# indianajohn/akaze-rust

Hardware: AMD Instinct MI355X
Metric: Mpix/s through extract_features (4 oct x 4 sub) (higher is better)
Workload: dtype f32

## Files before the change

### akaze-rust_amd/csrc/akz_api.cpp

```cpp
#include "akz_ctx.hpp"

unsigned akz::host_cpu_share() {
    unsigned n = std::max(1u, std::thread::hardware_concurrency());
    cpu_set_t set;
    if (sched_getaffinity(0, sizeof(set), &set) == 0) n = std::max(1, CPU_COUNT(&set));
    if (FILE* f = fopen("/sys/fs/cgroup/cpu.max", "r")) {
        char q[32] = {0};
        long period = 0;
        if (fscanf(f, "%31s %ld", q, &period) == 2 && period > 0 && strcmp(q, "max") != 0)
            n = std::min<unsigned>(n, (unsigned)std::max(1L, atol(q) / period));
        fclose(f);
    }
    if (const char* e = std::getenv("LOCAL_WORLD_SIZE")) {
        const int ranks = atoi(e);
        if (ranks > 1) n = std::max(2u, n / (unsigned)ranks);
    }
    return std::max(1u, n);
}

int level_info_out(const std::vector<LevelPlan>& plan, uint64_t level, double* etime, double* esigma,
                          uint32_t* octave, uint32_t* sublevel, uint32_t* sigma_size, uint32_t* lw, uint32_t* lh,
                          uint32_t* det_sigma, uint64_t* n_tau, double* tau, uint64_t tau_cap) {
    if (level >= plan.size()) {
        set_error("level out of range");
// ... 64 lines not shown
int akz_stream_create(int device, void** stream_out) {
    if (!stream_out) return AKZ_ERR_INVALID_ARG;
    AKZ_HIP_TRY(hipSetDevice(device));
    hipStream_t s = nullptr;
    AKZ_HIP_TRY(hipStreamCreateWithFlags(&s, hipStreamNonBlocking));
    *stream_out = (void*)s;
    return AKZ_OK;
}
int akz_stream_destroy(int device, void* stream) {
    AKZ_HIP_TRY(hipSetDevice(device));
    if (stream) AKZ_HIP_TRY(hipStreamDestroy((hipStream_t)stream));
    return AKZ_OK;
}

int akz_ctx_destroy(akz_ctx* c) {
    if (!c) return AKZ_OK;
    (void)hipSetDevice(c->device);
    finisher_stop(c);
    for (akz_ctx* l : c->lanes) (void)akz_ctx_destroy(l);
    c->lanes.clear();
    if (c->lane_in) { (void)hipEventDestroy(c->lane_in); c->lane_in = nullptr; }
    (void)hipStreamSynchronize(c->stream);
    DevBuf* bufs[] = {&c->lazy[0], &c->lazy[1], &c->lazy[2], &c->lazy[3], &c->lazy[4], &c->lazy[5],
                      &c->scratch[0], &c->scratch[1], &c->scratch[2], &c->scratch[3], &c->scratch[4], &c->scratch[5], &c->scratch_coarse,
                      &c->small, &c->cand, &c->cand_sorted, &c->sort_scratch, &c->rel_scratch, &c->sel_scratch, &c->sel_recs, &c->bucket_scratch, &c->kp_in, &c->kp_out, &c->match_a, &c->match_b, &c->match_rec, &c->match_state,
                      &c->match_out, &c->cosi, &c->mm_q8, &c->mm_t8, &c->mm_pop, &c->mm_tab, &c->mm_cols,
                      &c->ms1.q8, &c->ms1.t8, &c->ms1.pop, &c->ms1.tab, &c->ms1.cols, &c->ms1.rec, &c->ransac_dev,
                      &c->mp_in, &c->mp_raw, &c->mp_tab, &c->mp_trials, &c->mp_keep, &c->gd_tab, &c->gd_rec, &c->gd_out, &c->cx_rev, &c->kn_part, &c->kn_io};
    for (DevBuf* b : bufs)
        if (b->p) (void)hipFree(b->p);
    for (DevBuf* b : {&c->jpeg_coef, &c->jpeg_plane, &c->jpeg_frames})
        if (b->p) (void)hipFree(b->p);
    for (int k = 0; k < akz_ctx::kJpegSlots; ++k) {
        if (c->jpeg_up[k]) (void)hipEventDestroy(c->jpeg_up[k]);
        if (c->jpeg_pin[k].p) (void)hipHostFree(c->jpeg_pin[k].p);
    }
    for (DevBuf& b : c->fetch_tmp)
        if (b.p) (void)hipFree(b.p);
    for (auto& set : c->fetch_out)
        for (DevBuf& b : set)
            if (b.p) (void)hipFree(b.p);
    if (c->fetch_stage.p) (void)hipHostFree(c->fetch_stage.p);
    for (hipEvent_t* e : {&c->fetch_chunk[0], &c->fetch_chunk[1], &c->fetch_chunk[2], &c->fetch_chunk[3], &c->fetch_start,
                          &c->fetch_join, &c->fetch_ready[0], &c->fetch_ready[1], &c->fetch_free[0], &c->fetch_free[1]}) {
        if (*e) (void)hipEventDestroy(*e);
        *e = nullptr;
    }
// ... 274 lines not shown
int akz_ctx_set_candidate_hint(akz_ctx* c, uint32_t per_image) {
    AKZ_TRY(bind(c));
    c->cand_cap_hint = std::max<uint32_t>(per_image, 16u);
    for (akz_ctx* l : c->lanes) l->cand_cap_hint = c->cand_cap_hint.load();
    return AKZ_OK;
}
int akz_ctx_set_match_mode(akz_ctx* c, int mode) {
    AKZ_TRY(bind(c));
    if (mode < 0 || mode > 3) return AKZ_ERR_INVALID_ARG;
    c->match_mode = mode;
    for (akz_ctx* l : c->lanes) l->match_mode = mode;
    return AKZ_OK;
}
int akz_ctx_set_fed_mode(akz_ctx* c, int mode) {
    AKZ_TRY(bind(c));
    if (mode != 0 && mode != 2) return AKZ_ERR_INVALID_ARG;
    c->fed_mode = mode;
    for (akz_ctx* l : c->lanes) l->fed_mode = mode;
    return AKZ_OK;
}
const char* akz_fed_kernel_name(void) { return "k_level_march + k_fed_own"; }
int akz_debug_march_bands(int kind, uint32_t w, uint32_t h, uint32_t n, int half_width, int32_t* rows, uint32_t cap,
                          uint32_t* n_bands) {
    if (!n_bands || (cap && !rows) || kind < 0 || kind > 1 || w < 16 || h < 16 || n == 0 || half_width < 1 || half_width > 4)
        return AKZ_ERR_INVALID_ARG;
    *n_bands = launch::march_band_rows(kind, w, h, n, half_width, rows, cap);
    return AKZ_OK;
}
int akz_debug_detector_set_cells(int half_width, const uint32_t* w, const uint32_t* h, uint32_t n_entries, uint32_t n, int32_t* cells,
                                 uint32_t cap, int32_t* grids, uint32_t* n_workgroups) {
    if (!n_workgroups || !w || !h || !grids || (cap && !cells) || n_entries < 1 || n_entries > launch::detector_march_set_max() || n == 0 ||
        half_width < 1 || half_width > 4)
        return AKZ_ERR_INVALID_ARG;
    for (uint32_t e = 0; e < n_entries; ++e)
        if (w[e] < 4u * (uint32_t)half_width + 8u || h[e] < 4u * (uint32_t)half_width + 8u) return AKZ_ERR_INVALID_ARG;
    *n_workgroups = launch::detector_set_cells(half_width, w, h, n_entries, n, cells, cap, grids);
    return AKZ_OK;
}
const char* akz_detector_kernel_name(void) { return "detector (k_detector_march + k_detector_tiled)"; }
int akz_debug_set_schedule(akz_ctx* c, int key, int value) {
    if (!c || key < 0 || key > 11) return AKZ_ERR_INVALID_ARG;
    AKZ_TRY(bind(c));
    c->sched[key] = value;
    if (key == 7 || key == 8) launch::march_min_band_rows(c->sched[7], c->sched[8]);
    if (key == 11) launch::detector_set_waves(value >= 11 && value <= 14 ? value - 10 : 0);
    if (key == 4) {
        c->big_px_sync = value > 0 ? (uint64_t)value * 1000u : gates::kBigPxSync;
        c->big_px_async = value > 0 ? (uint64_t)value * 1000u : gates::kBigPxAsync;
        c->lane_px = value > 0 ? (uint64_t)value * 1000u : gates::kLanePx;
        for (akz_ctx* l : c->lanes) {
            l->big_px_sync = std::max(c->big_px_sync, c->lane_px);
            l->big_px_async = std::max(c->big_px_async, c->lane_px);
        }
    }
    return AKZ_OK;
}
int akz_debug_placement_verdict(float spin_pair_ms, float tiny_pair_ms, float tiny_alone_ms, float spin_ms) {
    return akz::placement_verdict(spin_pair_ms, tiny_pair_ms, tiny_alone_ms, spin_ms);
}
int akz_debug_stream_placement(akz_ctx* c, int* info) {
    if (!c || !info) return AKZ_ERR_INVALID_ARG;
    AKZ_TRY(bind(c));
    info[0] = c->placed ? 1 : 0;
    info[1] = c->pre_mode;
// ... 90 lines not shown
```

### akaze-rust_amd/csrc/akz_ctx.hpp

```cpp
#pragma once
#include <algorithm>
#include <cmath>
#include <cstdlib>
#include <cstddef>
#include <cstring>
#include <atomic>
#include <condition_variable>
#include <functional>
#include <map>
#include <memory>
#include <mutex>
#include <thread>
#include <sched.h>
#include <time.h>
#include <type_traits>

#include "akz_internal.hpp"
#include "akz_select.hpp"
#include "akz_pool.hpp"
#include "akz_gates.hpp"

#define AKZ_LOCAL __attribute__((visibility("hidden")))

namespace akz {
// ... 25 lines not shown
    bool quit = false;
};

enum Pin {
    PIN_LIST = 0,
    PIN_COUNT_SUMS,
    PIN_ROWS,
    PIN_PARAMS,
    PIN_COSI,
    PIN_CONTRAST,
    PIN_REL,
    PIN_REL_FLAGS,
    PIN_SEL_HDR,
    PIN_SPARE,
    PIN_COUNT_
};
struct akz_ctx {
    int device = 0;
    hipStream_t stream = nullptr;
    hipStream_t main = nullptr;
    bool own_stream = false;
    DevBuf scratch[6];
    DevBuf scratch_coarse;
    DevBuf lazy[6];
    DevBuf small;
    void* small_zero_p = nullptr;
    size_t small_zero = 0;
    DevBuf cand;
    DevBuf cand_sorted, sort_scratch;
    DevBuf rel_scratch;
    DevBuf sel_scratch, sel_recs;
    DevBuf bucket_scratch;
    int dbg_select = -1;
    std::atomic<uint32_t> last_total_kp{0};
    std::atomic<int> sel_last_mode{-1};
    std::atomic<int> sel_skip{0};
    std::atomic<uint64_t> sel_skip_shape{0};
    std::atomic<uint32_t> sel_last_ticks[4];
    std::atomic<uint32_t> sel_last_rounds{0}, sel_last_fallback{0};
    DevBuf kp_in, kp_out;
    DevBuf match_a, match_b, match_rec, match_out;
    DevBuf match_state;
    uint32_t match_epoch = 0;
    DevBuf ransac_dev, ransac_pin;
    DevBuf mp_in, mp_raw, mp_tab, mp_trials, mp_keep;
    DevBuf mp_pin_in, mp_pin_tab, mp_pin_smp[2], mp_pin_out;
// ... 34 lines not shown
    std::atomic<uint32_t> cand_cap_hint{1u << 15};
    std::atomic<int> live_results{0};
    bool dead = false;
    std::atomic<uint32_t> last_total_cands{0};
    std::atomic<uint64_t> last_cand_shape{0};
    hipStream_t aux = nullptr;
    std::mutex aux_m;
    hipStream_t coarse = nullptr;
    hipStream_t pre = nullptr;
    hipEvent_t pre_done = nullptr;
    hipStream_t copy = nullptr;
    DevBuf stage[kSlots];
    hipEvent_t staged[kSlots] = {nullptr, nullptr, nullptr};
    std::vector<akz_ctx*> lanes;
    unsigned next_lane = 0;
    bool is_lane = false;
    bool eager_finish = true;
    std::shared_ptr<Finisher> fin;
    hipEvent_t lane_in = nullptr;
    uint64_t stream_min_px = gates::kStreamPx;
    int prep_mode = 2;
    int det_mode = 2;
    int fed_mode = 2;
    int sched[12] = {0, 1, 0, 0, 0, 0, 0, 0, 0, 0, 0, 0};
    uint64_t big_px = gates::kBigPxAsync;
    uint64_t big_px_sync = gates::kBigPxSync, big_px_async = gates::kBigPxAsync;
    uint64_t lane_px = gates::kLanePx;
    static constexpr uint64_t kLaunchMarchPx = gates::kMarchPx;
    uint64_t launch_min_px = kLaunchMarchPx;
    bool placed = false;
    int pre_mode = 0;
    int place_replaced = 0;
    int place_collisions = 0;
    int place_retries = 0;
    int lane_collisions = 0;
    hipEvent_t probe_ev[2] = {nullptr, nullptr};
    int profiling = 0;
    akz_profile prof{};
    struct Span { int stage; hipEvent_t a, b; int row; };
    std::vector<Span> spans;
    std::vector<akz_kernel_row> rows;
    std::vector<hipEvent_t> ev_pool;
    std::mutex ev_m;
    static constexpr int kFedRing = 4;
    hipEvent_t fed_ev[kFedRing] = {nullptr, nullptr, nullptr, nullptr};
    hipEvent_t pre_ev[kFedRing] = {nullptr, nullptr, nullptr, nullptr};
    std::atomic<uint64_t> begin_seq{0};
// ... 276 lines not shown
```

### akaze-rust_amd/csrc/akz_extract_begin.cpp

```cpp
#include "akz_extract.hpp"

namespace {
enum class Prep : uint8_t {
    Tiled,
    Stream,
    LevelMarch,
    Resident
};
enum class Det : uint8_t {
    Fallback,
    NmsFused,
    TiledSet,
    March
};
struct BeginRoute {
    bool big = false;
    int prep_mode = 0;
    int pre_on = 0;
    bool level1_clone = false;
    size_t res_first = 0;
    size_t fork_level = 0;
    size_t oct1 = 0;
    bool own_kernels = true;
    struct Level {
        Prep prep = Prep::Tiled;
        uint32_t n1 = 0, rem = 0;
        bool fold_half = false;
        bool may_ride = false;
        Det det = Det::Fallback;
    };
    std::vector<Level> lv;
};

BeginRoute begin_route(const akz_ctx* c, const std::vector<LevelPlan>& plan, const akz_config& cfg, uint32_t w, uint32_t h, uint32_t n,
                       uint32_t flags, bool input_ready, bool big) {
    const size_t L = plan.size();
    BeginRoute rt;
    rt.big = big;
    rt.prep_mode = c->prep_mode;
    rt.lv.resize(L);
    const int pre_mode = c->sched[0] == 0 ? c->pre_mode : c->sched[0] == 1 ? 2 : c->sched[0] == 2 ? 1 : 0;
    if ((input_ready || (flags & AKZ_INPUT_READY)) && pre_mode != 0 && c->profiling < 2 && c->prep_mode == 2 && big &&
        launch::blur5_march_supported(w, h, (uint32_t)gaussian_kernel_size((float)cfg.base_scale_offset)) &&
        launch::contrast_march_supported(w, h, (uint32_t)gaussian_kernel_size(1.0f), (uint32_t)cfg.contrast_factor_num_bins))
        rt.pre_on = pre_mode;
    rt.level1_clone = L > 1 && plan[1].octave == plan[0].octave && plan[1].w == w && plan[1].h == h;
    const int fork_octave = c->sched[3] > 0 ? c->sched[3] : 2;
    rt.res_first = L;
    if (c->fed_mode == 2 && (c->prep_mode == 3 || (c->prep_mode == 2 && big))) {
        size_t f = 1;
// ... 24 lines not shown
        const LevelPlan& lv = plan[l];
        BeginRoute::Level& q = rt.lv[l];
        const int fam = detector_family(c, lv.det_sigma, lv.w, lv.h, n, border_margin(lv, cfg), (flags & AKZ_KEEP_ALL_PLANES) != 0);
        q.det = fam == 5 ? Det::March : fam == 4 ? Det::TiledSet : launch::detector_nms_fused_supported(lv.det_sigma) ? Det::NmsFused : Det::Fallback;
        if (l >= rt.fork_level && q.det == Det::Fallback) rt.own_kernels = false;
        if (l == 0) continue;
        const LevelPlan& pv = plan[l - 1];
        const bool half = lv.octave > pv.octave;
        const uint64_t lpx = (uint64_t)lv.w * lv.h * n;
        if (l >= rt.res_first) {
            q.prep = Prep::Resident;
        } else if (!lv.tau.empty() && c->fed_mode == 2 && launch::level_march_supported(lv.w, lv.h) &&
                   (c->prep_mode == 3 || (c->prep_mode == 2 && lpx >= gates::kLevelMarchPx))) {
            q.prep = Prep::LevelMarch;
            q.n1 = std::min<uint32_t>((uint32_t)lv.tau.size(), 4u);
            q.rem = (uint32_t)lv.tau.size() - q.n1;
            q.fold_half = half && launch::level_march_half_supported(lv.w, lv.h, pv.w, pv.h, q.n1);
        } else if (c->prep_mode != 0 && launch::prep_stream_supported(lv.w, lv.h) &&
                   (c->prep_mode == 1 || (c->prep_mode >= 2 && !half && lpx >= c->stream_min_px))) {
            q.prep = Prep::Stream;
        }
        q.may_ride = c->sched[6] == 0 && c->fed_mode == 2 && lv.octave == pv.octave && q.prep == Prep::Tiled;
    }
    return rt;
}

struct BeginState {
    akz_ctx* c;
    akz_result* r;
    const BeginRoute& rt;
    uint32_t n;
    bool keep_all;
    hipStream_t s;
    hipStream_t ls;
    uint64_t seq;
    Candidate* d_cand;
    uint32_t* d_count;
    uint32_t cap;
    std::vector<float> g1;
    std::vector<char> det_done;
    std::vector<char> prepared;
    bool head_fused = false;
    float* P(size_t l, int p) const { return r->planes[l][p]; }
    size_t L() const { return r->plan.size(); }
};

// ... 70 lines not shown
                                           (uint32_t)plan[l].tau.size(), ht[l].data(), plan[l].octave});
        px_steps += (uint64_t)plan[l].w * plan[l].h * b.n * plan[l].tau.size();
    }
    StageTimer st(c, AKZ_ST_FED);
    st.kernel(AKZ_KR_OCTAVE_RESIDENT, (uint32_t)rl.size(), plan[i].w, plan[i].h, b.n, 1, 0, px_steps);
    launch::octave_resident(b.ls, b.P(i - 1, AKZ_LT), plan[i - 1].w, plan[i - 1].h, b.n, rl.data(), (uint32_t)rl.size(), b.g1.data(), b.r->d_k);
    if (c->profiling) {
        c->prof.fed_launches += 1;
        c->prof.fed_px_steps += px_steps;
    }
    AKZ_HIP_TRY(hipGetLastError());
    return AKZ_OK;
}

int level_by_march(BeginState& b, size_t i, float* A, float* B) {
    akz_ctx* c = b.c;
    const LevelPlan &lv = b.r->plan[i], &pv = b.r->plan[i - 1];
    const BeginRoute::Level& q = b.rt.lv[i];
    const uint32_t n = b.n, n1 = q.n1, rem = q.rem;
    const bool half = lv.octave > pv.octave;
    const uint32_t rest = rem ? fed_num_launches(c, rem, lv.w, lv.h, n) : 0;
    float* d1 = fed_dst(rest + 1, 1, A, B);
    const float* level_in = b.P(i - 1, AKZ_LT);
    if (half && !q.fold_half) {
        StageTimer st(c, AKZ_ST_PREP);
        float* hb = d1 == A ? B : A;
        launch::half_size(b.ls, b.P(i - 1, AKZ_LT), hb, pv.w, pv.h, n);
        level_in = hb;
    }
    float ht[4];
    for (uint32_t j = 0; j < n1; ++j) ht[j] = 0.5f * (float)lv.tau[j];
    {
        StageTimer st(c, AKZ_ST_FED);
        st.kernel(AKZ_KR_LEVEL_MARCH, n1 | (q.fold_half ? 16u : 0u) | ((rem == 0 && b.keep_all) ? 32u : 0u), lv.w, lv.h, n, 1,
                  (uint64_t)lv.w * lv.h * n, (uint64_t)lv.w * lv.h * n * n1);
        launch::level_march(b.ls, level_in, b.P(i, AKZ_LSMOOTH), b.P(i, AKZ_LFLOW), d1,
                            (rem == 0 && b.keep_all) ? b.P(i, AKZ_LSTEP) : nullptr, lv.w, lv.h, n, b.g1.data(), b.r->d_k,
                            lv.octave, ht, n1, q.fold_half ? pv.w : 0u, q.fold_half ? pv.h : 0u);
        if (c->profiling) {
            c->prof.fed_launches += 1;
            c->prof.fed_px_steps += (uint64_t)lv.w * lv.h * n * n1;
            c->prof.fused_px += (uint64_t)lv.w * lv.h * n;
        }
    }
    if (rem) {
        StageTimer st(c, AKZ_ST_FED);
        st.kernel(AKZ_KR_FED_OWN, rem, lv.w, lv.h, n, rest, 0, (uint64_t)lv.w * lv.h * n * rem);
        AKZ_TRY(fed_impl(c, d1, A, B, b.P(i, AKZ_LFLOW), b.keep_all ? b.P(i, AKZ_LSTEP) : nullptr, lv.w, lv.h, n, lv.tau.data() + n1, rem));
    }
    AKZ_HIP_TRY(hipGetLastError());
    return AKZ_OK;
}

int level_by_launches(BeginState& b, size_t i, float* A, float* B) {
    akz_ctx* c = b.c;
    const LevelPlan &lv = b.r->plan[i], &pv = b.r->plan[i - 1];
    const uint32_t n = b.n, n_tau = (uint32_t)lv.tau.size();
    const bool half = lv.octave > pv.octave;
    const float* fed_in = b.P(i - 1, AKZ_LT);
    float* half_buf = nullptr;
    if (half) {
// ... 184 lines not shown
    if (!c->fed_ev[0])
        for (hipEvent_t& e : c->fed_ev) AKZ_HIP_TRY(hipEventCreateWithFlags(&e, hipEventDisableTiming));
    if (!c->pre_ev[0])
        for (hipEvent_t& e : c->pre_ev) AKZ_HIP_TRY(hipEventCreateWithFlags(&e, hipEventDisableTiming));
    const uint64_t seq = c->begin_seq.load() + 1;
    struct StreamRestore {
        akz_ctx* c;
        hipStream_t main;
        ~StreamRestore() { c->stream = main; }
    } stream_restore{c, s};
    struct PrepModeRestore {
        akz_ctx* c;
        int mode;
        ~PrepModeRestore() { c->prep_mode = mode; }
    } prep_mode_restore{c, c->prep_mode};
    if (c->prep_mode == 2 && c->sched[6] == 0 && (uint64_t)w * h * n < gates::kTiledPrepPx) c->prep_mode = 0;
    const bool big = (uint64_t)w * h * n >= c->big_px;
    c->launch_min_px = big ? std::min<uint64_t>(akz_ctx::kLaunchMarchPx, (uint64_t)w * h * n) : akz_ctx::kLaunchMarchPx;
    if (big && !c->placed) AKZ_TRY(place_streams(c));
    const BeginRoute rt = begin_route(c, r->plan, r->cfg, w, h, n, flags, input_ready != nullptr, big);
    BeginState b{c, r, rt, n, keep_all, s, s, seq, (Candidate*)c->cand_slot[o.slot].p, (uint32_t*)c->count_slot[o.slot].p, cap,
                 {}, std::vector<char>(L, 0), std::vector<char>(L + 1, 0)};

    AKZ_TRY(level0<T>(b, d_imgs, input_ready));
    AKZ_TRY(ensure(c, c->scratch[5], plane_bytes(w, h, n)));
    b.g1 = gaussian_kernel(1.0f, gaussian_kernel_size(1.0f));
    AKZ_TRY(run_levels(b, 1, rt.oct1));
    AKZ_HIP_TRY(hipEventRecord(c->pre_ev[seq % akz_ctx::kFedRing], s));
    AKZ_TRY(run_levels(b, rt.oct1, rt.fork_level));
    AKZ_HIP_TRY(hipEventRecord(c->fed_ev[seq % akz_ctx::kFedRing], s));
    c->begin_seq.store(seq);

    hipStream_t done_on = s;
    if (rt.fork_level < L) AKZ_TRY(fork_and_join(b, &done_on));
    else AKZ_TRY(detectors(b, 0, L, s));
    AKZ_HIP_TRY(hipGetLastError());
    job->nms_done = StageTimer::get(c);
    AKZ_HIP_TRY(hipEventRecord(job->nms_done, done_on));
    job->done_stream = done_on;
    job->seq = seq;
    *out = o.keep(cap);
    return AKZ_OK;
}
template int extract_begin<uint8_t>(akz_ctx*, const uint8_t*, uint32_t, uint32_t, uint32_t, const akz_config*, uint32_t, akz_job**, int, hipEvent_t, bool);
template int extract_begin<float>(akz_ctx*, const float*, uint32_t, uint32_t, uint32_t, const akz_config*, uint32_t, akz_job**, int, hipEvent_t, bool);
```

### akaze-rust_amd/csrc/akz_internal.hpp

```cpp
#pragma once
#include <hip/hip_runtime.h>

#include <cstdint>
#include <functional>
#include <string>
#include <vector>

#include "../../include/akaze_hip.h"
#include "../../include/akaze_hip_debug.h"

namespace akz {

void set_error(const std::string& msg);
unsigned host_cpu_share();

using TrialsOnDevice = std::function<int(const float*, const float*, const float*, const float*, uint32_t, const uint32_t*, uint32_t,
                                         float, float, float*, int32_t*)>;
int remove_outliers_impl(const akz_keypoint* keypoints_0, uint64_t n0, const akz_keypoint* keypoints_1, uint64_t n1,
                         const akz_match* matches, uint64_t n_matches, uint64_t num_trials, float epsilon_model,
                         float epsilon_inlier, akz_match* out, uint64_t* n_out, const TrialsOnDevice& trials_on_device);

#define AKZ_HIP_TRY(expr)                                                                          \
    do {                                                                                           \
        hipError_t _e = (expr);                                                                    \
// ... 183 lines not shown
void detector_march(hipStream_t s, const float* lsmooth, uint32_t sigma, float* lx, float* ly, float* lxx, float* lyy,
                    float* lxy, float* ldet_out, uint32_t w, uint32_t h, uint32_t n, uint32_t level, float thr,
                    float border_m, Candidate* d_cand, uint32_t cap, uint32_t* d_count);
uint32_t detector_march_set_max();
void detector_march_set(hipStream_t s, uint32_t sigma, const DetLevelDesc* levels, uint32_t nlevels, uint32_t n, float thr,
                        Candidate* d_cand, uint32_t cap, uint32_t* d_count);
void detector_set_waves(int waves);
uint32_t detector_set_cells(int S, const uint32_t* w, const uint32_t* h, uint32_t nlv, uint32_t n, int32_t* cells, uint32_t cap,
                            int32_t* grids);
bool head_fused_supported(uint32_t w, uint32_t h, uint32_t ntaps0, uint32_t ntaps1);
void head_fused_u8(hipStream_t s, const uint8_t* in, float* lt0, float* blurred, float* gx, float* gy, uint32_t w, uint32_t h, uint32_t n,
                   const float* k5, const float* g3, unsigned long long* d_smax_bits, uint32_t* d_zero_word = nullptr);
void head_fused_f32(hipStream_t s, const float* in, float* lt0, float* blurred, float* gx, float* gy, uint32_t w, uint32_t h, uint32_t n,
                    const float* k5, const float* g3, unsigned long long* d_smax_bits, uint32_t* d_zero_word = nullptr);
void contrast_hist_final(hipStream_t s, const float* gx, const float* gy, uint32_t w, uint32_t h, uint32_t n, unsigned long long* d_smax_bits,
                         uint32_t nbins, uint32_t* d_hist, uint32_t* d_done, double percentile, double* d_k);
void flow_from_pair(hipStream_t s, const float* gx, const float* gy, float* lflow, uint32_t w, uint32_t h, uint32_t n, const double* d_k,
                    uint32_t k_pow);
void march_min_band_rows(int detector, int level);
bool level_march_supported(uint32_t w, uint32_t h);
bool level_march_half_supported(uint32_t w, uint32_t h, uint32_t pw, uint32_t ph, uint32_t n_steps);
void level_march(hipStream_t s, const float* prev, float* lsmooth, float* lflow, float* lt_out, float* lstep, uint32_t w,
                 uint32_t h, uint32_t n, const float* g3, const double* d_k, uint32_t k_pow, const float* half_taus,
                 uint32_t n_steps, uint32_t pw = 0, uint32_t ph = 0);
struct ResidentLevel {
    float *lt, *lsmooth, *lflow, *lstep;
    uint32_t w, h;
    bool half;
    uint32_t n_tau;
    const float* half_tau;
    uint32_t k_pow;
};
constexpr int kResidentMaxLevels = 10;
constexpr int kResidentMaxSteps = 448;
bool octave_resident_supported(uint32_t w, uint32_t h);
void octave_resident(hipStream_t s, const float* prev, uint32_t pw, uint32_t ph, uint32_t n, const ResidentLevel* levels,
                     uint32_t n_levels, const float* g3, const double* d_k);
bool detector_nms_fused_supported(uint32_t sigma);
void detector_nms_fused(hipStream_t s, const float* lsmooth, uint32_t sigma, float* lx, float* ly, float* lxx,
                        float* lyy, float* lxy, float* ldet_out, uint32_t w, uint32_t h, uint32_t n, uint32_t level,
                        float thr, float border_m, Candidate* d_cand, uint32_t cap, uint32_t* d_count);
void rcp_f64_to_f32(hipStream_t s, const double* x, float* out, uint64_t n);
void accumulate(hipStream_t s, float* a, const float* b, uint64_t count);
void ldet(hipStream_t s, const float* lxx, const float* lyy, const float* lxy, float* out, uint64_t count,
          float sigma_quat);
size_t sort_candidates_scratch(uint32_t cap, uint64_t max_px, uint32_t n_levels, uint32_t n_images);
uint32_t sort_small_capacity();
// ... 154 lines not shown
```

### akaze-rust_amd/csrc/akz_march.hip

```cpp
#include <hip/hip_runtime.h>

#include <algorithm>
#include <cstdlib>
#include <type_traits>

#include "akz_internal.hpp"
#include "akz_pm_g2.hpp"

namespace akz {
namespace {

typedef float f2 __attribute__((ext_vector_type(2)));
typedef float f2u __attribute__((ext_vector_type(2), aligned(4)));

constexpr int MT = 256;
constexpr int MW = 2 * MT;
constexpr int HALO = 16;
constexpr int USE = MW - 2 * HALO;
constexpr int PAD = 8;
constexpr int ROW = MW + 2 * PAD;
constexpr int CBUF = 32;
#ifndef AKZ_MARCH_PF
#define AKZ_MARCH_PF 3
#endif
// ... 373 lines not shown
        }
    }
    if (NMS) cands_flush(cbuf, cnum, nms, lane);
}

struct LevelTaus {
    float half_tau[4];
};
__device__ __forceinline__ f2 lds2(const float* p) { return f2{p[0], p[1]}; }
__device__ __forceinline__ f2 tap3(f2 a, f2 b, f2 c, float k0, float k1, float k2) {
    const f2 z = {0.0f, 0.0f};
    return ((z + k0 * a) + k1 * b) + k2 * c;
}
__device__ __forceinline__ double octave_contrast(double k, unsigned pow) {
    for (unsigned i = 0; i < pow; ++i) k = k * 0.75;
    return k;
}

typedef unsigned u4m __attribute__((ext_vector_type(4)));
template <int N, bool KEEPSTEP, bool ODDW, bool HALF = false>
__global__ void __launch_bounds__(MT, 3)
k_level_march(const float* __restrict__ prev, float* __restrict__ lsmooth_out, float* __restrict__ lflow_out,
              float* __restrict__ lt_out, float* __restrict__ lstep_out, int w, int h, MarchGrid g, float g0, float g1,
              float g2, float kn, float kwn, const double* __restrict__ d_k, unsigned k_pow, LevelTaus ht, int pw = 0, int ph = 0) {
    static_assert(!(HALF && ODDW), "the 2x2 mean is folded in for even level widths only");
    static_assert(N >= 1 && N <= 4, "fused diffusion steps");
    static_assert(N + 3 <= HALO, "strip halo");
    constexpr int NPL = 3 + N;
#ifndef AKZ_LEVEL_PF
#define AKZ_LEVEL_PF 2
#endif
    constexpr int PF = AKZ_LEVEL_PF;
    static_assert(PF >= 1 && PF <= 3, "prefetch ring");
    __shared__ __attribute__((aligned(16))) float s_row[2][NPL][ROW];
    const int tid = threadIdx.x;
    const int per = g.nbands * g.nstrips;
    const int cell = march_cell();
    if (cell >= g.total) return;
    const int img = __builtin_amdgcn_readfirstlane(cell / per);
    const int rem = cell - img * per;
    const int band = __builtin_amdgcn_readfirstlane(rem / g.nstrips), strip = rem - band * g.nstrips;
    int cs, ce;
    level_band_rows(g, band, h, &cs, &ce);
    if (cs >= ce) return;
    const int lt0 = cs == 1 ? 0 : cs, lt1 = ce == h - 1 ? h : ce;

    const int X0 = strip * USE - HALO;
    const int p0 = (2 * tid + HALO) & (MW - 1);
    const bool inner = p0 >= HALO && p0 < MW - HALO;
    const Cols C = make_cols(X0 + p0, inner, w);
    const int i0 = PAD + clampi(clampi(C.x0, 1, w - 2) - X0, 0, MW - 1) - 1;
    const int i1 = PAD + clampi(clampi(C.x0 + 1, 1, w - 2) - X0, 0, MW - 1) - 1;
    const int wi = PAD + p0;
    const bool edge_h = __ballot(i0 != wi - 1 || i1 != wi) != 0ull;
    const bool hxn0 = C.x0 > 0, hxp0 = C.x0 + 1 < w, hxn1 = C.x0 + 1 > 0, hxp1 = C.x0 + 2 < w;
    const bool edge_col = __ballot(!(hxn0 && hxp0 && hxn1 && hxp1)) != 0ull;

    const size_t base = (size_t)img * (size_t)w * (size_t)h;
    const __amdgpu_buffer_rsrc_t in = HALF ? plane_rsrc(prev + (size_t)img * (size_t)pw * (size_t)ph, pw, ph) : plane_rsrc(prev + base, w, h);
    const __amdgpu_buffer_rsrc_t o_ls[1] = {plane_rsrc(lsmooth_out + base, w, h)};
    const __amdgpu_buffer_rsrc_t o_lf[1] = {plane_rsrc(lflow_out + base, w, h)};
    __amdgpu_buffer_rsrc_t o_lt[KEEPSTEP ? 2 : 1];
    o_lt[0] = plane_rsrc(lt_out + base, w, h);
    if (KEEPSTEP) o_lt[1] = plane_rsrc(lstep_out + base, w, h);
    const __amdgpu_buffer_rsrc_t(&o_ltc)[KEEPSTEP ? 2 : 1] = o_lt;
    const double kc = octave_contrast(d_k[img], k_pow);
    const double inverse_k = 1.0 / (kc * kc);

    const int v0 = lt0 - N - 2;
    const int T = (lt1 - lt0) + 2 * N + 6;
    struct Fed {
        f2 v;
        u4m top, bot;
    };
    auto feed = [&](int t) -> Fed {
        Fed f;
        const unsigned row = (unsigned)clampi(v0 + min(t, T - 1), 0, h - 1);
        if constexpr (HALF) {
            const unsigned ro = 2u * row * ((unsigned)pw * 4u);
            f.top = __builtin_amdgcn_raw_buffer_load_b128(in, (int)(2u * C.vo_ld), (int)ro, 0);
            f.bot = __builtin_amdgcn_raw_buffer_load_b128(in, (int)(2u * C.vo_ld), (int)(ro + (unsigned)pw * 4u), 0);
        } else {
            f.v = load_pair<ODDW>(in, row * ((unsigned)w * 4u), C);
        }
        return f;
    };
    auto pair_of = [&](const Fed& f) -> f2 {
        if constexpr (HALF) {
// ... 123 lines not shown
                    } else {
                        tx.x = hxp0 ? (hxn0 ? XFE.x - XFW.x : XFE.x) : -XFW.x;
                        tx.y = hxp1 ? (hxn1 ? XFE.y - XFW.y : XFE.y) : -XFW.y;
                    }
                    f2 tt;
                    if (MID || r + 1 < h) {
                        tt = tx + SV * (Lp - Lc);
                        if (MID || r > 0) tt = tt - SU * (Lc - Lm);
                    } else {
                        tt = tx + SU * (Lm - Lc);
                    }
                    st = ht.half_tau[s - 1] * tt;
                    lnew = Lc + st;
                }
                {
                    const int r = v - 4 - N;
                    {
                        f2 o[KEEPSTEP ? 2 : 1];
                        o[0] = lnew;
                        if constexpr (KEEPSTEP) o[1] = st;
                        const f2(&oc)[KEEPSTEP ? 2 : 1] = o;
                        store_rows<KEEPSTEP ? 2 : 1, ODDW>(o_ltc, r, w, r >= lt0 && r < lt1, C, oc);
                    }
                }
                ls_c = ls_n;
                lf_c = lf_n;
            }
        }
    }
    };
    const int v_last = v0 + ((T + 7) & ~7) - 1;
    if (v0 >= N + 5 && v_last <= h - 2) rows(std::true_type{});
    else rows(std::false_type{});
}

struct ContrastMarchArgs {
    unsigned long long* hmax_bits;
    unsigned* hist;
    unsigned nbins;
    const double* thr;
};
constexpr int CM_COPIES = 2;
template <int MODE, bool ODDW>
__global__ void __launch_bounds__(MT, 8)
k_contrast_march(const float* __restrict__ in_plane, int w, int h, MarchGrid g, float g0, float g1, float g2, float kn,
                 float kwn, ContrastMarchArgs ca) {
// ... 246 lines not shown
namespace launch {
static int g_det_min_rows = 0, g_lvl_min_rows = 0, g_head_min_rows = 0;
void march_min_band_rows(int detector, int level) {
    g_det_min_rows = detector;
    g_lvl_min_rows = level % 1000;
    g_head_min_rows = level / 1000;
}
}
namespace {
using launch::g_det_min_rows;
using launch::g_lvl_min_rows;
using launch::g_head_min_rows;

inline int march_cus() {
    static int cus = 0;
    if (!cus) {
        int dev = 0;
        hipDeviceProp_t p;
        if (hipGetDevice(&dev) == hipSuccess && hipGetDeviceProperties(&p, dev) == hipSuccess) cus = p.multiProcessorCount;
        if (cus <= 0) cus = 256;
    }
    return cus;
}
inline MarchGrid plan_level_march(uint32_t w, uint32_t h, uint32_t n, dim3* grid, int fill_wg = 3, int min_band_rows = 64) {
    const int cus = march_cus();
    const int fill = fill_wg, min_rows = min_band_rows;
    MarchGrid g;
    g.nstrips = (int)((w + USE - 1) / USE);
    const int rows = (int)h - 2;
    const long cols = (long)n * g.nstrips;
    const long want = ((long)cus * fill + cols - 1) / cols;
    long nb = std::max<long>(1, std::min<long>(want, std::max(1, rows / min_rows)));
    constexpr int edge_pct = 75;
    if (nb >= 3) {
        const double m = (double)rows / ((double)(nb - 2) + 2.0 * edge_pct / 100.0);
        g.band_rows = std::max(1, (int)(m + 0.999));
        g.edge_rows = std::max(1, (int)((rows - (long)(nb - 2) * g.band_rows) / 2));
        g.nbands = (int)nb;
        if (g.edge_rows + (long)(nb - 2) * g.band_rows >= rows) {
            g.band_rows = (int)((rows + nb - 1) / nb);
            g.edge_rows = g.band_rows;
            g.nbands = (rows + g.band_rows - 1) / g.band_rows;
        }
    } else {
        g.band_rows = (int)((rows + nb - 1) / nb);
        g.edge_rows = g.band_rows;
        g.nbands = (rows + g.band_rows - 1) / g.band_rows;
    }
    g.total = (int)(cols * g.nbands);
    *grid = dim3((unsigned)((g.total + 7) / 8 * 8));
    return g;
}

inline MarchGrid plan_march(uint32_t w, uint32_t h, uint32_t n, int S, dim3* grid, int fill_wg = 3, int min_band_rows = 64) {
    const int cus = march_cus();
    const int fill = fill_wg, min_rows = min_band_rows;
    const int use = USE;
    (void)S;
    MarchGrid g;
    g.nstrips = (int)((w + use - 1) / use);
    const int rows = (int)h - 2 * S;
    const long cols = (long)n * g.nstrips;
    const long want = ((long)cus * fill + cols - 1) / cols;
    long nb = std::max<long>(1, std::min<long>(want, std::max(1, rows / min_rows)));
    g.band_rows = (int)((rows + nb - 1) / nb);
    g.edge_rows = g.band_rows;
    g.nbands = (rows + g.band_rows - 1) / g.band_rows;
    g.total = (int)(cols * g.nbands);
    *grid = dim3((unsigned)((g.total + 7) / 8 * 8));
    return g;
}
// ... 172 lines not shown
    dim3 gr;
    const MarchGrid mg = plan_level_march(w, h, n, &gr, 8, g_head_min_rows > 0 ? g_head_min_rows : 32);
    if (w & 1u)
        hipLaunchKernelGGL((k_contrast_march<1, true>), gr, dim3(MT), 0, s, in, (int)w, (int)h, mg, g3[0], g3[1], g3[2], m.wgt[0], m.wgt[1], ca);
    else
        hipLaunchKernelGGL((k_contrast_march<1, false>), gr, dim3(MT), 0, s, in, (int)w, (int)h, mg, g3[0], g3[1], g3[2], m.wgt[0], m.wgt[1], ca);
    contrast_thresholds(s, d_hmax_bits, nbins, n, d_thr);
    const size_t lds = ((size_t)(MT / 64) * CM_COPIES * nbins) * sizeof(unsigned) + (size_t)(nbins + 1) * sizeof(double);
    if (w & 1u)
        hipLaunchKernelGGL((k_contrast_march<2, true>), gr, dim3(MT), lds, s, in, (int)w, (int)h, mg, g3[0], g3[1], g3[2], m.wgt[0], m.wgt[1], ca);
    else
        hipLaunchKernelGGL((k_contrast_march<2, false>), gr, dim3(MT), lds, s, in, (int)w, (int)h, mg, g3[0], g3[1], g3[2], m.wgt[0], m.wgt[1], ca);
}

#ifndef AKZ_LVL_FILL
#define AKZ_LVL_FILL 3
#endif
static int level_min_band_rows(uint32_t w, uint32_t h, uint32_t n) {
    if (g_lvl_min_rows > 0) return g_lvl_min_rows;
    return (uint64_t)w * h * n < (48u << 20) ? 20 : 64;
}
uint32_t march_band_rows(int kind, uint32_t w, uint32_t h, uint32_t n, int S, int32_t* cs_ce, uint32_t cap) {
    dim3 gr;
    const MarchGrid g = kind == 1 ? plan_level_march(w, h, n, &gr, AKZ_LVL_FILL, level_min_band_rows(w, h, n)) : plan_march(w, h, n, S, &gr);
    for (int b = 0; b < g.nbands && (uint32_t)b < cap; ++b) {
        int cs, ce;
        if (kind == 1) level_band_rows(g, b, (int)h, &cs, &ce);
        else uniform_band_rows(g, b, S, (int)h, &cs, &ce);
        cs_ce[2 * b] = cs;
        cs_ce[2 * b + 1] = ce;
    }
    return (uint32_t)g.nbands;
}

bool level_march_supported(uint32_t w, uint32_t h) { return w >= 16 && h >= 16 && (uint64_t)w * h <= (1ull << 28); }

template <int NS, bool KEEPSTEP>
static void launch_level_march(hipStream_t s, dim3 gr, const MarchGrid& mg, const float* prev, float* lsmooth, float* lflow,
                               float* lt_out, float* lstep, uint32_t w, uint32_t h, const float* g3, const Taps& m,
                               const double* d_k, uint32_t k_pow, const LevelTaus& ht, uint32_t pw, uint32_t ph) {
    if constexpr (NS == 4) {
        if (pw) {
            hipLaunchKernelGGL((k_level_march<NS, KEEPSTEP, false, true>), gr, dim3(MT), 0, s, prev, lsmooth, lflow, lt_out, lstep, (int)w,
                               (int)h, mg, g3[0], g3[1], g3[2], m.wgt[0], m.wgt[1], d_k, k_pow, ht, (int)pw, (int)ph);
            return;
        }
    }
    if (w & 1u)
        hipLaunchKernelGGL((k_level_march<NS, KEEPSTEP, true>), gr, dim3(MT), 0, s, prev, lsmooth, lflow, lt_out, lstep, (int)w,
                           (int)h, mg, g3[0], g3[1], g3[2], m.wgt[0], m.wgt[1], d_k, k_pow, ht);
    else
        hipLaunchKernelGGL((k_level_march<NS, KEEPSTEP, false>), gr, dim3(MT), 0, s, prev, lsmooth, lflow, lt_out, lstep, (int)w,
                           (int)h, mg, g3[0], g3[1], g3[2], m.wgt[0], m.wgt[1], d_k, k_pow, ht);
}
#define AKZ_LEVEL(NS)                                                                                                        \
    case NS: {                                                                                                               \
        if (lstep) launch_level_march<NS, true>(s, gr, mg, prev, lsmooth, lflow, lt_out, lstep, w, h, g3, m, d_k, k_pow, ht, pw, ph);  \
        else launch_level_march<NS, false>(s, gr, mg, prev, lsmooth, lflow, lt_out, lstep, w, h, g3, m, d_k, k_pow, ht, pw, ph);       \
    } break;

bool level_march_half_supported(uint32_t w, uint32_t h, uint32_t pw, uint32_t ph, uint32_t n_steps) {
    return n_steps == 4 && (pw & 3u) == 0 && (w & 1u) == 0 && w == pw / 2 && h == ph / 2 && (uint64_t)pw * ph <= (1ull << 28);
}
void level_march(hipStream_t s, const float* prev, float* lsmooth, float* lflow, float* lt_out, float* lstep, uint32_t w,
                 uint32_t h, uint32_t n, const float* g3, const double* d_k, uint32_t k_pow, const float* half_taus,
                 uint32_t n_steps, uint32_t pw, uint32_t ph) {
    const Taps m = taps_scharr_main(1);
    LevelTaus ht;
    for (uint32_t i = 0; i < 4; ++i) ht.half_tau[i] = i < n_steps ? half_taus[i] : 0.0f;
    dim3 gr;
    const MarchGrid mg = plan_level_march(w, h, n, &gr, AKZ_LVL_FILL, level_min_band_rows(w, h, n));
    switch (n_steps) {
        AKZ_LEVEL(1) AKZ_LEVEL(2) AKZ_LEVEL(3) AKZ_LEVEL(4)
        default: break;
    }
}
#undef AKZ_LEVEL

}
}
```

Before: 15210.

## Emit half-size downsample from level march at octave boundaries

The last level march of each octave now writes the 2x2-mean half-resolution plane directly from registers into a new scratch buffer. The first level of the next octave reads that buffer instead of folding the downsample into its own march. Band rows are forced to even boundaries so each workgroup owns whole row pairs. The intent is to avoid re-reading the full-resolution previous level, at the cost of extra stores, a new buffer, and adjusted band planning. It can be disabled through a new schedule key.

```diff
diff --git a/akaze-rust_amd/csrc/akz_api.cpp b/akaze-rust_amd/csrc/akz_api.cpp
--- a/akaze-rust_amd/csrc/akz_api.cpp
+++ b/akaze-rust_amd/csrc/akz_api.cpp
@@ -110,7 +110,7 @@
     if (c->lane_in) { (void)hipEventDestroy(c->lane_in); c->lane_in = nullptr; }
     (void)hipStreamSynchronize(c->stream);
     DevBuf* bufs[] = {&c->lazy[0], &c->lazy[1], &c->lazy[2], &c->lazy[3], &c->lazy[4], &c->lazy[5],
-                      &c->scratch[0], &c->scratch[1], &c->scratch[2], &c->scratch[3], &c->scratch[4], &c->scratch[5], &c->scratch_coarse,
+                      &c->scratch[0], &c->scratch[1], &c->scratch[2], &c->scratch[3], &c->scratch[4], &c->scratch[5], &c->scratch_coarse, &c->scratch_half,
                       &c->small, &c->cand, &c->cand_sorted, &c->sort_scratch, &c->rel_scratch, &c->sel_scratch, &c->sel_recs, &c->bucket_scratch, &c->kp_in, &c->kp_out, &c->match_a, &c->match_b, &c->match_rec, &c->match_state,
                       &c->match_out, &c->cosi, &c->mm_q8, &c->mm_t8, &c->mm_pop, &c->mm_tab, &c->mm_cols,
                       &c->ms1.q8, &c->ms1.t8, &c->ms1.pop, &c->ms1.tab, &c->ms1.cols, &c->ms1.rec, &c->ransac_dev,
@@ -431,7 +431,7 @@
 const char* akz_fed_kernel_name(void) { return "k_level_march + k_fed_own"; }
 int akz_debug_march_bands(int kind, uint32_t w, uint32_t h, uint32_t n, int half_width, int32_t* rows, uint32_t cap,
                           uint32_t* n_bands) {
-    if (!n_bands || (cap && !rows) || kind < 0 || kind > 1 || w < 16 || h < 16 || n == 0 || half_width < 1 || half_width > 4)
+    if (!n_bands || (cap && !rows) || kind < 0 || kind > 2 || w < 16 || h < 16 || n == 0 || half_width < 1 || half_width > 4)
         return AKZ_ERR_INVALID_ARG;
     *n_bands = launch::march_band_rows(kind, w, h, n, half_width, rows, cap);
     return AKZ_OK;
@@ -448,7 +448,7 @@
 }
 const char* akz_detector_kernel_name(void) { return "detector (k_detector_march + k_detector_tiled)"; }
 int akz_debug_set_schedule(akz_ctx* c, int key, int value) {
-    if (!c || key < 0 || key > 11) return AKZ_ERR_INVALID_ARG;
+    if (!c || key < 0 || key > 12) return AKZ_ERR_INVALID_ARG;
     AKZ_TRY(bind(c));
     c->sched[key] = value;
     if (key == 7 || key == 8) launch::march_min_band_rows(c->sched[7], c->sched[8]);
diff --git a/akaze-rust_amd/csrc/akz_ctx.hpp b/akaze-rust_amd/csrc/akz_ctx.hpp
--- a/akaze-rust_amd/csrc/akz_ctx.hpp
+++ b/akaze-rust_amd/csrc/akz_ctx.hpp
@@ -71,6 +71,7 @@
     bool own_stream = false;
     DevBuf scratch[6];
     DevBuf scratch_coarse;
+    DevBuf scratch_half;
     DevBuf lazy[6];
     DevBuf small;
     void* small_zero_p = nullptr;
@@ -151,7 +152,7 @@
     int prep_mode = 2;
     int det_mode = 2;
     int fed_mode = 2;
-    int sched[12] = {0, 1, 0, 0, 0, 0, 0, 0, 0, 0, 0, 0};
+    int sched[13] = {0, 1, 0, 0, 0, 0, 0, 0, 0, 0, 0, 0, 0};
     uint64_t big_px = gates::kBigPxAsync;
     uint64_t big_px_sync = gates::kBigPxSync, big_px_async = gates::kBigPxAsync;
     uint64_t lane_px = gates::kLanePx;
diff --git a/akaze-rust_amd/csrc/akz_extract_begin.cpp b/akaze-rust_amd/csrc/akz_extract_begin.cpp
--- a/akaze-rust_amd/csrc/akz_extract_begin.cpp
+++ b/akaze-rust_amd/csrc/akz_extract_begin.cpp
@@ -26,6 +26,8 @@
         Prep prep = Prep::Tiled;
         uint32_t n1 = 0, rem = 0;
         bool fold_half = false;
+        bool half_out = false;
+        bool half_in = false;
         bool may_ride = false;
         Det det = Det::Fallback;
     };
@@ -96,6 +98,15 @@
         }
         q.may_ride = c->sched[6] == 0 && c->fed_mode == 2 && lv.octave == pv.octave && q.prep == Prep::Tiled;
     }
+    for (size_t l = 1; l + 1 < L && l + 1 < rt.fork_level; ++l) {
+        BeginRoute::Level &q = rt.lv[l], &nx = rt.lv[l + 1];
+        if (c->sched[12] == 0 && plan[l + 1].octave > plan[l].octave && q.prep == Prep::LevelMarch && nx.prep == Prep::LevelMarch && q.rem == 0 &&
+            nx.fold_half && launch::level_march_half_out_supported(plan[l].w, plan[l].h)) {
+            q.half_out = true;
+            nx.half_in = true;
+            nx.fold_half = false;
+        }
+    }
     return rt;
 }
 
@@ -212,7 +223,9 @@
     const uint32_t rest = rem ? fed_num_launches(c, rem, lv.w, lv.h, n) : 0;
     float* d1 = fed_dst(rest + 1, 1, A, B);
     const float* level_in = b.P(i - 1, AKZ_LT);
-    if (half && !q.fold_half) {
+    if (q.half_in) {
+        level_in = (const float*)c->scratch_half.p;
+    } else if (half && !q.fold_half) {
         StageTimer st(c, AKZ_ST_PREP);
         float* hb = d1 == A ? B : A;
         launch::half_size(b.ls, b.P(i - 1, AKZ_LT), hb, pv.w, pv.h, n);
@@ -222,11 +235,11 @@
     for (uint32_t j = 0; j < n1; ++j) ht[j] = 0.5f * (float)lv.tau[j];
     {
         StageTimer st(c, AKZ_ST_FED);
-        st.kernel(AKZ_KR_LEVEL_MARCH, n1 | (q.fold_half ? 16u : 0u) | ((rem == 0 && b.keep_all) ? 32u : 0u), lv.w, lv.h, n, 1,
+        st.kernel(AKZ_KR_LEVEL_MARCH, n1 | (q.fold_half ? 16u : 0u) | ((rem == 0 && b.keep_all) ? 32u : 0u) | (q.half_out ? 64u : 0u), lv.w, lv.h, n, 1,
                   (uint64_t)lv.w * lv.h * n, (uint64_t)lv.w * lv.h * n * n1);
         launch::level_march(b.ls, level_in, b.P(i, AKZ_LSMOOTH), b.P(i, AKZ_LFLOW), d1,
                             (rem == 0 && b.keep_all) ? b.P(i, AKZ_LSTEP) : nullptr, lv.w, lv.h, n, b.g1.data(), b.r->d_k,
-                            lv.octave, ht, n1, q.fold_half ? pv.w : 0u, q.fold_half ? pv.h : 0u);
+                            lv.octave, ht, n1, q.fold_half ? pv.w : 0u, q.fold_half ? pv.h : 0u, q.half_out ? (float*)c->scratch_half.p : nullptr);
         if (c->profiling) {
             c->prof.fed_launches += 1;
             c->prof.fed_px_steps += (uint64_t)lv.w * lv.h * n * n1;
@@ -457,6 +470,8 @@
     BeginState b{c, r, rt, n, keep_all, s, s, seq, (Candidate*)c->cand_slot[o.slot].p, (uint32_t*)c->count_slot[o.slot].p, cap,
                  {}, std::vector<char>(L, 0), std::vector<char>(L + 1, 0)};
 
+    for (size_t l = 1; l < L; ++l)
+        if (rt.lv[l].half_out) AKZ_TRY(ensure(c, c->scratch_half, plane_bytes(r->plan[l].w / 2, r->plan[l].h / 2, n)));
     AKZ_TRY(level0<T>(b, d_imgs, input_ready));
     AKZ_TRY(ensure(c, c->scratch[5], plane_bytes(w, h, n)));
     b.g1 = gaussian_kernel(1.0f, gaussian_kernel_size(1.0f));
diff --git a/akaze-rust_amd/csrc/akz_internal.hpp b/akaze-rust_amd/csrc/akz_internal.hpp
--- a/akaze-rust_amd/csrc/akz_internal.hpp
+++ b/akaze-rust_amd/csrc/akz_internal.hpp
@@ -229,7 +229,8 @@
 bool level_march_half_supported(uint32_t w, uint32_t h, uint32_t pw, uint32_t ph, uint32_t n_steps);
 void level_march(hipStream_t s, const float* prev, float* lsmooth, float* lflow, float* lt_out, float* lstep, uint32_t w,
                  uint32_t h, uint32_t n, const float* g3, const double* d_k, uint32_t k_pow, const float* half_taus,
-                 uint32_t n_steps, uint32_t pw = 0, uint32_t ph = 0);
+                 uint32_t n_steps, uint32_t pw = 0, uint32_t ph = 0, float* half_out = nullptr);
+bool level_march_half_out_supported(uint32_t w, uint32_t h);
 struct ResidentLevel {
     float *lt, *lsmooth, *lflow, *lstep;
     uint32_t w, h;
diff --git a/akaze-rust_amd/csrc/akz_march.hip b/akaze-rust_amd/csrc/akz_march.hip
--- a/akaze-rust_amd/csrc/akz_march.hip
+++ b/akaze-rust_amd/csrc/akz_march.hip
@@ -419,7 +419,8 @@
 __global__ void __launch_bounds__(MT, 3)
 k_level_march(const float* __restrict__ prev, float* __restrict__ lsmooth_out, float* __restrict__ lflow_out,
               float* __restrict__ lt_out, float* __restrict__ lstep_out, int w, int h, MarchGrid g, float g0, float g1,
-              float g2, float kn, float kwn, const double* __restrict__ d_k, unsigned k_pow, LevelTaus ht, int pw = 0, int ph = 0) {
+              float g2, float kn, float kwn, const double* __restrict__ d_k, unsigned k_pow, LevelTaus ht, int pw = 0, int ph = 0,
+              float* __restrict__ half_out = nullptr) {
     static_assert(!(HALF && ODDW), "the 2x2 mean is folded in for even level widths only");
     static_assert(N >= 1 && N <= 4, "fused diffusion steps");
     static_assert(N + 3 <= HALO, "strip halo");
@@ -461,6 +462,8 @@
     o_lt[0] = plane_rsrc(lt_out + base, w, h);
     if (KEEPSTEP) o_lt[1] = plane_rsrc(lstep_out + base, w, h);
     const __amdgpu_buffer_rsrc_t(&o_ltc)[KEEPSTEP ? 2 : 1] = o_lt;
+    const __amdgpu_buffer_rsrc_t o_half = plane_rsrc(half_out + (size_t)img * (size_t)(w >> 1) * (size_t)(h >> 1), w >> 1, half_out ? h >> 1 : 0);
+    f2 lt_even = {0.0f, 0.0f};
     const double kc = octave_contrast(d_k[img], k_pow);
     const double inverse_k = 1.0 / (kc * kc);
 
@@ -630,6 +633,16 @@
                         const f2(&oc)[KEEPSTEP ? 2 : 1] = o;
                         store_rows<KEEPSTEP ? 2 : 1, ODDW>(o_ltc, r, w, r >= lt0 && r < lt1, C, oc);
                     }
+                    if constexpr (!ODDW && !HALF) {
+                        if ((k & 1) == 0) {
+                            lt_even = lnew;
+                        } else if (half_out != nullptr && r >= lt0 && r < lt1) {
+                            float a = 0.0f;
+                            a = a + lt_even.x; a = a + lnew.x; a = a + lt_even.y; a = a + lnew.y;
+                            __builtin_amdgcn_raw_buffer_store_b32(__float_as_uint(a / 4.0f), o_half, (int)(C.vo_st >> 1),
+                                                                  (int)((unsigned)(r >> 1) * ((unsigned)(w >> 1) * 4u)), 0);
+                        }
+                    }
                 }
                 ls_c = ls_n;
                 lf_c = lf_n;
@@ -922,7 +935,8 @@
     }
     return cus;
 }
-inline MarchGrid plan_level_march(uint32_t w, uint32_t h, uint32_t n, dim3* grid, int fill_wg = 3, int min_band_rows = 64) {
+inline MarchGrid plan_level_march(uint32_t w, uint32_t h, uint32_t n, dim3* grid, int fill_wg = 3, int min_band_rows = 64,
+                                  bool pair_rows = false) {
     const int cus = march_cus();
     const int fill = fill_wg, min_rows = min_band_rows;
     MarchGrid g;
@@ -947,6 +961,11 @@
         g.edge_rows = g.band_rows;
         g.nbands = (rows + g.band_rows - 1) / g.band_rows;
     }
+    if (pair_rows && g.nbands > 1) {
+        g.band_rows += g.band_rows & 1;
+        g.edge_rows |= 1;
+        g.nbands = g.edge_rows >= rows ? 1 : 1 + (rows - g.edge_rows + g.band_rows - 1) / g.band_rows;
+    }
     g.total = (int)(cols * g.nbands);
     *grid = dim3((unsigned)((g.total + 7) / 8 * 8));
     return g;
@@ -1165,10 +1184,10 @@
 }
 uint32_t march_band_rows(int kind, uint32_t w, uint32_t h, uint32_t n, int S, int32_t* cs_ce, uint32_t cap) {
     dim3 gr;
-    const MarchGrid g = kind == 1 ? plan_level_march(w, h, n, &gr, AKZ_LVL_FILL, level_min_band_rows(w, h, n)) : plan_march(w, h, n, S, &gr);
+    const MarchGrid g = kind >= 1 ? plan_level_march(w, h, n, &gr, AKZ_LVL_FILL, level_min_band_rows(w, h, n), kind == 2) : plan_march(w, h, n, S, &gr);
     for (int b = 0; b < g.nbands && (uint32_t)b < cap; ++b) {
         int cs, ce;
-        if (kind == 1) level_band_rows(g, b, (int)h, &cs, &ce);
+        if (kind >= 1) level_band_rows(g, b, (int)h, &cs, &ce);
         else uniform_band_rows(g, b, S, (int)h, &cs, &ce);
         cs_ce[2 * b] = cs;
         cs_ce[2 * b + 1] = ce;
@@ -1181,38 +1200,40 @@
 template <int NS, bool KEEPSTEP>
 static void launch_level_march(hipStream_t s, dim3 gr, const MarchGrid& mg, const float* prev, float* lsmooth, float* lflow,
                                float* lt_out, float* lstep, uint32_t w, uint32_t h, const float* g3, const Taps& m,
-                               const double* d_k, uint32_t k_pow, const LevelTaus& ht, uint32_t pw, uint32_t ph) {
+                               const double* d_k, uint32_t k_pow, const LevelTaus& ht, uint32_t pw, uint32_t ph, float* half_out) {
     if constexpr (NS == 4) {
         if (pw) {
             hipLaunchKernelGGL((k_level_march<NS, KEEPSTEP, false, true>), gr, dim3(MT), 0, s, prev, lsmooth, lflow, lt_out, lstep, (int)w,
-                               (int)h, mg, g3[0], g3[1], g3[2], m.wgt[0], m.wgt[1], d_k, k_pow, ht, (int)pw, (int)ph);
+                               (int)h, mg, g3[0], g3[1], g3[2], m.wgt[0], m.wgt[1], d_k, k_pow, ht, (int)pw, (int)ph, nullptr);
             return;
         }
     }
     if (w & 1u)
         hipLaunchKernelGGL((k_level_march<NS, KEEPSTEP, true>), gr, dim3(MT), 0, s, prev, lsmooth, lflow, lt_out, lstep, (int)w,
-                           (int)h, mg, g3[0], g3[1], g3[2], m.wgt[0], m.wgt[1], d_k, k_pow, ht);
+                           (int)h, mg, g3[0], g3[1], g3[2], m.wgt[0], m.wgt[1], d_k, k_pow, ht, 0, 0, nullptr);
     else
         hipLaunchKernelGGL((k_level_march<NS, KEEPSTEP, false>), gr, dim3(MT), 0, s, prev, lsmooth, lflow, lt_out, lstep, (int)w,
-                           (int)h, mg, g3[0], g3[1], g3[2], m.wgt[0], m.wgt[1], d_k, k_pow, ht);
+                           (int)h, mg, g3[0], g3[1], g3[2], m.wgt[0], m.wgt[1], d_k, k_pow, ht, 0, 0, half_out);
 }
 #define AKZ_LEVEL(NS)                                                                                                        \
     case NS: {                                                                                                               \
-        if (lstep) launch_level_march<NS, true>(s, gr, mg, prev, lsmooth, lflow, lt_out, lstep, w, h, g3, m, d_k, k_pow, ht, pw, ph);  \
-        else launch_level_march<NS, false>(s, gr, mg, prev, lsmooth, lflow, lt_out, lstep, w, h, g3, m, d_k, k_pow, ht, pw, ph);       \
+        if (lstep) launch_level_march<NS, true>(s, gr, mg, prev, lsmooth, lflow, lt_out, lstep, w, h, g3, m, d_k, k_pow, ht, pw, ph, half_out);  \
+        else launch_level_march<NS, false>(s, gr, mg, prev, lsmooth, lflow, lt_out, lstep, w, h, g3, m, d_k, k_pow, ht, pw, ph, half_out);       \
     } break;
 
 bool level_march_half_supported(uint32_t w, uint32_t h, uint32_t pw, uint32_t ph, uint32_t n_steps) {
     return n_steps == 4 && (pw & 3u) == 0 && (w & 1u) == 0 && w == pw / 2 && h == ph / 2 && (uint64_t)pw * ph <= (1ull << 28);
 }
+bool level_march_half_out_supported(uint32_t w, uint32_t h) { return (w & 3u) == 0 && h >= 2 && level_march_supported(w, h); }
 void level_march(hipStream_t s, const float* prev, float* lsmooth, float* lflow, float* lt_out, float* lstep, uint32_t w,
                  uint32_t h, uint32_t n, const float* g3, const double* d_k, uint32_t k_pow, const float* half_taus,
-                 uint32_t n_steps, uint32_t pw, uint32_t ph) {
+                 uint32_t n_steps, uint32_t pw, uint32_t ph, float* half_out) {
+    if (half_out && (pw || !level_march_half_out_supported(w, h))) return;
     const Taps m = taps_scharr_main(1);
     LevelTaus ht;
     for (uint32_t i = 0; i < 4; ++i) ht.half_tau[i] = i < n_steps ? half_taus[i] : 0.0f;
     dim3 gr;
-    const MarchGrid mg = plan_level_march(w, h, n, &gr, AKZ_LVL_FILL, level_min_band_rows(w, h, n));
+    const MarchGrid mg = plan_level_march(w, h, n, &gr, AKZ_LVL_FILL, level_min_band_rows(w, h, n), half_out != nullptr);
     switch (n_steps) {
         AKZ_LEVEL(1) AKZ_LEVEL(2) AKZ_LEVEL(3) AKZ_LEVEL(4)
         default: break;
```

After: 15260 (median of 4 runs). Within noise of the previous version (+0.3%).
